# NthPortal/reservoir

Measured on AMD Instinct MI355X. Metric: elements sampled/sec (Gelem/s) + % HBM roofline, 1B Long keys k=1024, 1/2/4/8 GPU, higher is better.
Workload: dtype int64

## Files before the change

reservoir_amd/csrc/rsv_elements.hip:

```cpp
#include <algorithm>

#include "rsv_device.h"
#include "rsv_internal.h"
#include "rsv_scan.h"

namespace rsv {

namespace {

constexpr int kBlock = 256;

constexpr int kK1Unroll = 2;

constexpr unsigned kK1Grid = 256 * 20;

constexpr int kK1Win = 12;
struct K1Lds {
    uint64_t q[kBlock / 64][k1q_cap<kK1Win>()];
    uint64_t cq[kBlock / 64][kQueue];
};

__device__ __forceinline__ bool k1_fast(uint64_t lo, uint64_t hi) {
    return (lo >> 33) == ((hi - 1) >> 33) && hi <= (1ull << 40);
}

struct K1Sched {
    uint32_t W1, A, B;
};

__global__ __launch_bounds__(kBlock) void k1_last_writer(DrawKey dk, uint32_t k, uint64_t lo,
                                                         uint64_t hi, uint64_t g_begin,
                                                         uint64_t n_groups,
                                                         unsigned long long* __restrict__ win, K1Sched sch) {
    __shared__ K1Lds L;
    const int w = threadIdx.x >> 6;
    if (k1_fast(lo, hi))
        k1_body_q<kK1Win, true>(dk, k, lo, hi, g_begin, n_groups, win, L.q[w], L.cq[w], sch.W1, sch.A, sch.B);
    else
        k1_body_q<kK1Win, false>(dk, k, lo, hi, g_begin, n_groups, win, L.q[w], L.cq[w], sch.W1, sch.A, sch.B);
}

template <typename Take, typename Empty, typename Keep>
__device__ __forceinline__ void slot_rule(int64_t j, unsigned long long wi, int64_t base, int64_t n, int fresh,
                                          Take&& take, Empty&& empty, Keep&& keep) {
    if (wi) take((int64_t)wi - base, (int64_t)wi, true);
    else if (j >= base && j < base + n) take(j - base, j, false);
    else if (fresh) empty((int64_t)-1);
    else keep();
}

template <typename KeyT, int R, bool kAgentWin>
__device__ __forceinline__ void resolve_registers_first(const KeyT* __restrict__ keys, int64_t base, int64_t n,
                                                        uint32_t k, unsigned long long* __restrict__ win,
                                                        KeyT* __restrict__ slot_key, int64_t* __restrict__ slot_idx,
                                                        int fresh, int64_t m, KeyT* dst, uint32_t* flag, uint32_t gen) {
    unsigned long long wi[R];
    KeyT v[R];
#pragma unroll
    for (int r = 0; r < R; ++r) {
        const uint32_t j = threadIdx.x + r * kBlock;
        if (j >= k) wi[r] = 0ull;
        else if (kAgentWin) wi[r] = __hip_atomic_load(&win[j], __ATOMIC_RELAXED, __HIP_MEMORY_SCOPE_AGENT);
        else wi[r] = win[j];
    }
#pragma unroll
    for (int r = 0; r < R; ++r) {
        const int64_t j = threadIdx.x + r * kBlock;
        if (j >= k) continue;
        KeyT x;
        slot_rule(
            j, wi[r], base, n, fresh, [&](int64_t off, int64_t, bool) { x = keys[off]; }, [&](int64_t) { x = 0; },
            [&] { x = slot_key[j]; });
        v[r] = x;
    }
#pragma unroll
    for (int r = 0; r < R; ++r) {
        const int64_t j = threadIdx.x + r * kBlock;
        if (j >= k) continue;
        const KeyT x = v[r];
        slot_rule(
            j, wi[r], base, n, fresh,
            [=](int64_t, int64_t idx, bool winner) {
                slot_key[j] = x;
                slot_idx[j] = idx;
                if (winner) win[j] = 0;
            },
            [=](int64_t idx) {
                slot_key[j] = 0;
                slot_idx[j] = idx;
            },
            [] {});
        if (j < m) dst[j] = x;
    }
    publish_flag(flag, gen);
}

constexpr uint32_t kK1FusedMaxK = 8 * kBlock;

template <typename KeyT>
__global__ __launch_bounds__(kBlock) void k1_resolve_publish(DrawKey dk, uint32_t k, uint64_t lo, uint64_t hi,
                                                             uint64_t g_begin, uint64_t n_groups,
                                                             unsigned long long* __restrict__ win,
                                                             uint32_t* ticket, const KeyT* __restrict__ keys,
                                                             int64_t base, int64_t n, KeyT* __restrict__ slot_key,
                                                             int64_t* __restrict__ slot_idx, int fresh, int64_t m,
                                                             KeyT* dst, uint32_t* flag, uint32_t gen, K1Sched sch) {
    __shared__ K1Lds L;
    __shared__ uint32_t last;
    const int w = threadIdx.x >> 6;
    if (k1_fast(lo, hi))
        k1_body_q<kK1Win, true>(dk, k, lo, hi, g_begin, n_groups, win, L.q[w], L.cq[w], sch.W1, sch.A, sch.B);
    else
        k1_body_q<kK1Win, false>(dk, k, lo, hi, g_begin, n_groups, win, L.q[w], L.cq[w], sch.W1, sch.A, sch.B);
    asm volatile("s_waitcnt vmcnt(0)" ::: "memory");
    __syncthreads();
    if (threadIdx.x == 0) {
        const uint32_t prev = __hip_atomic_fetch_add(ticket, 1u, __ATOMIC_RELAXED, __HIP_MEMORY_SCOPE_AGENT);
        last = prev == gridDim.x - 1;
        if (last) __hip_atomic_store(ticket, 0u, __ATOMIC_RELAXED, __HIP_MEMORY_SCOPE_AGENT);
    }
    __syncthreads();
    if (!last) return;
    __builtin_amdgcn_fence(__ATOMIC_ACQUIRE, "agent");
    resolve_registers_first<KeyT, kK1FusedMaxK / kBlock, true>(keys, base, n, k, win, slot_key, slot_idx, fresh, m, dst,
                                                               flag, gen);
}

template <typename KeyT, bool kPublish>
__global__ __launch_bounds__(kPublish ? 1024 : kBlock) void resolve_kernel(const KeyT* __restrict__ keys, int64_t base,
                                                                         int64_t n, uint32_t k,
                                                                         unsigned long long* __restrict__ win,
                                                                         KeyT* __restrict__ slot_key,
                                                                         int64_t* __restrict__ slot_idx, int fresh,
                                                                         int64_t m, KeyT* dst, uint32_t* flag,
                                                                         uint32_t gen) {
    const uint32_t stride = gridDim.x * blockDim.x;
    for (uint32_t j = blockIdx.x * blockDim.x + threadIdx.x; j < k; j += stride) {
        KeyT v = 0;
        slot_rule(
            j, win[j], base, n, fresh,
            [&](int64_t off, int64_t idx, bool winner) {
                slot_key[j] = v = keys[off];
                if (kPublish || slot_idx) slot_idx[j] = idx;
                if (winner) win[j] = 0;
            },
            [=](int64_t idx) {
                slot_key[j] = 0;
                if (kPublish || slot_idx) slot_idx[j] = idx;
            },
            [&] {
                if (kPublish) v = slot_key[j];
            });
        if (kPublish && (int64_t)j < m) dst[j] = v;
    }
    if (kPublish) publish_flag(flag, gen);
}

template <typename KeyT, int R>
__global__ __launch_bounds__(kBlock) void resolve_publish_small_kernel(const KeyT* __restrict__ keys, int64_t base,
                                                                       int64_t n, uint32_t k,
                                                                       unsigned long long* __restrict__ win,
                                                                       KeyT* __restrict__ slot_key,
                                                                       int64_t* __restrict__ slot_idx, int fresh,
                                                                       int64_t m, KeyT* dst, uint32_t* flag, uint32_t gen) {
    resolve_registers_first<KeyT, R, false>(keys, base, n, k, win, slot_key, slot_idx, fresh, m, dst, flag, gen);
}

__global__ __launch_bounds__(kBlock) void replay_kernel(const int64_t* __restrict__ ev_pos,
                                                        const int32_t* __restrict__ ev_slot,
                                                        int64_t n_events, uint32_t k,
                                                        unsigned long long* __restrict__ win) {
    const int64_t e = (int64_t)blockIdx.x * blockDim.x + threadIdx.x;
    if (e >= n_events) return;
    const int32_t s = ev_slot[e];
    const int64_t p = ev_pos[e];
    if (s >= 0 && (uint32_t)s < k && p >= 2) atomicMax(&win[s], (unsigned long long)(p - 1));
}

__global__ __launch_bounds__(kBlock) void export_draws_kernel(DrawKey dk, uint64_t i0, int64_t n,
                                                              uint64_t* __restrict__ out) {
    const int64_t t = (int64_t)blockIdx.x * blockDim.x + threadIdx.x;
    if (t >= n) return;
    const uint64_t i = i0 + (uint64_t)t;
    const u32x4 w = level0(dk, i >> 4);
    out[t] = exact_j(dk, i, level0_byte(w, (uint32_t)(i & 15)));
}

template <typename KeyT>
struct StridedParts {
    using Key = KeyT;
    const int64_t* idx;
    const KeyT* key;
    int64_t part_len;
    __device__ int64_t index(int32_t p, uint32_t j) const { return idx[(int64_t)p * part_len + j]; }
    __device__ void take(int32_t p, uint32_t j, KeyT* slot_key) const { slot_key[j] = key[(int64_t)p * part_len + j]; }
};

template <typename KeyT>
struct PackedRows {
    using Key = KeyT;
    const int64_t* rows;
    int64_t stride;
    uint32_t k;
    __device__ int64_t index(int32_t p, uint32_t j) const { return rows[(int64_t)p * stride + j]; }
    __device__ void take(int32_t p, uint32_t j, KeyT* slot_key) const {
        slot_key[j] = (KeyT)rows[(int64_t)p * stride + k + j];
    }
};

struct StridedWideParts {
    using Key = uint32_t;
    const int64_t* idx;
    const uint32_t* key;
    int64_t part_len;
    uint32_t words;
    __device__ int64_t index(int32_t p, uint32_t j) const { return idx[(int64_t)p * part_len + j]; }
    __device__ void take(int32_t p, uint32_t j, uint32_t* slot_key) const {
        const uint32_t* src = key + ((size_t)p * part_len + j) * words;
        for (uint32_t q = 0; q < words; ++q) slot_key[(size_t)j * words + q] = src[q];
    }
};

struct PackedWideRows {
    using Key = uint32_t;
    const int64_t* rows;
    int64_t stride;
    uint32_t k, words;
    __device__ int64_t index(int32_t p, uint32_t j) const { return rows[(int64_t)p * stride + j]; }
    __device__ void take(int32_t p, uint32_t j, uint32_t* slot_key) const {
        const uint32_t* src = (const uint32_t*)(rows + (int64_t)p * stride + k) + (size_t)j * words;
        for (uint32_t q = 0; q < words; ++q) slot_key[(size_t)j * words + q] = src[q];
    }
};

template <typename Src>
__device__ __forceinline__ int32_t merge_winner(const Src& src, int32_t parts, uint32_t j, int64_t& best) {
    int32_t from = -1;
    for (int32_t p = 0; p < parts; ++p) {
        const int64_t idx = src.index(p, j);
        if (idx > best) {
            best = idx;
            from = p;
        }
    }
    return from;
}

template <typename Src, bool kPublish>
__global__ __launch_bounds__(kPublish ? 1024 : kBlock) void merge_kernel(Src src, int32_t parts, uint32_t k,
                                                                       int64_t* __restrict__ slot_idx,
                                                                       typename Src::Key* __restrict__ slot_key,
                                                                       int64_t m, typename Src::Key* dst,
                                                                       uint32_t* flag, uint32_t gen) {
    const uint32_t stride = gridDim.x * blockDim.x;
    for (uint32_t j = blockIdx.x * blockDim.x + threadIdx.x; j < k; j += stride) {
        int64_t best = slot_idx[j];
        const int32_t from = merge_winner(src, parts, j, best);
        if (from >= 0) {
            slot_idx[j] = best;
            src.take(from, j, slot_key);
        }
        if (kPublish && (int64_t)j < m) dst[j] = slot_key[j];
    }
    if (kPublish) publish_flag(flag, gen);
}

template <typename KeyT>
__global__ __launch_bounds__(kBlock) void export_packed_kernel(const int64_t* __restrict__ slot_idx,
                                                               const KeyT* __restrict__ slot_key, uint32_t k,
                                                               int64_t* __restrict__ row) {
    const uint32_t j = blockIdx.x * blockDim.x + threadIdx.x;
    if (j >= k) return;
    row[j] = slot_idx[j];
    row[k + j] = (int64_t)slot_key[j];
}

__global__ __launch_bounds__(1024) void resolve_wide_kernel(const uint32_t* __restrict__ keys, int64_t base,
                                                            int64_t n, uint32_t k, uint32_t words,
                                                            unsigned long long* __restrict__ win,
                                                            uint32_t* __restrict__ slot_key,
                                                            int64_t* __restrict__ slot_idx, int fresh, int64_t m,
                                                            uint32_t* dst, uint32_t* flag, uint32_t gen) {
    const uint32_t stride = gridDim.x * blockDim.x;
    for (uint32_t j = blockIdx.x * blockDim.x + threadIdx.x; j < k; j += stride) {
        const uint32_t* src = nullptr;
        bool write = true;
        slot_rule(
            j, win[j], base, n, fresh,
            [&](int64_t off, int64_t idx, bool winner) {
                src = keys + (size_t)off * words;
                slot_idx[j] = idx;
                if (winner) win[j] = 0;
            },
            [=](int64_t idx) { slot_idx[j] = idx; }, [&] { write = false; });
        uint32_t* o = slot_key + (size_t)j * words;
        const bool out = dst && (int64_t)j < m;
        for (uint32_t q = 0; q < words; ++q) {
            const uint32_t v = src ? src[q] : (write ? 0u : o[q]);
            if (write) o[q] = v;
            if (out) dst[(size_t)j * words + q] = v;
        }
    }
    if (dst) publish_flag(flag, gen);
}

__global__ __launch_bounds__(kBlock) void export_packed_wide_kernel(const int64_t* __restrict__ slot_idx,
                                                                    const uint32_t* __restrict__ slot_key, uint32_t k,
                                                                    uint32_t words, int64_t* __restrict__ row) {
    const uint32_t j = blockIdx.x * blockDim.x + threadIdx.x;
    if (j >= k) return;
    row[j] = slot_idx[j];
    uint32_t* o = (uint32_t*)(row + k) + (size_t)j * words;
    for (uint32_t q = 0; q < words; ++q) o[q] = slot_key[(size_t)j * words + q];
}

inline DrawKey make_key(const DrawParams& dp) {
    return DrawKey{(uint32_t)dp.seed, (uint32_t)(dp.seed >> 32), (uint32_t)dp.stream,
                   (uint32_t)(dp.stream >> 32)};
}

inline unsigned grid_for(uint64_t items, unsigned cap = ~0u) {
    uint64_t b = (items + kBlock - 1) / kBlock;
    if (b < 1) b = 1;
    return (unsigned)(b < cap ? b : cap);
}

inline unsigned k1_grid(uint64_t n_groups) {
    constexpr uint64_t per_window = (uint64_t)kK1Unroll * kBlock * kK1Win;
    if (n_groups < per_window * 768) return grid_for((n_groups + kK1Unroll - 1) / kK1Unroll, kK1Grid);
    const uint64_t m = std::max<uint64_t>(1, (n_groups + per_window * kK1Grid / 2) / (per_window * kK1Grid));
    return (unsigned)std::max<uint64_t>(1, n_groups / (per_window * m));
}

constexpr uint32_t kK1W1 = 256 * 6 * (kBlock / 64);
inline unsigned k1_plan(uint64_t n_groups, K1Sched& sch) {
    sch = K1Sched{0, 0, 0};
    constexpr uint64_t UB = (uint64_t)kK1Unroll * 64 * (kK1Win / 2);
    const uint64_t units = (n_groups + UB - 1) / UB;
    const uint64_t A = (units * 755 / 1000 + kK1W1 / 2) / kK1W1;
    if (n_groups < (uint64_t)kK1Unroll * kBlock * kK1Win * 768 || A < 10) return k1_grid(n_groups);
    sch.W1 = kK1W1;
    sch.A = (uint32_t)A;
    sch.B = 2;
    const uint64_t rest = units - (uint64_t)kK1W1 * A;
    const uint64_t waves = kK1W1 + (rest + sch.B - 1) / sch.B;
    return (unsigned)((waves + kBlock / 64 - 1) / (kBlock / 64));
}

template <typename F>
hipError_t with_key_type(int key_width, F&& f) {
    if (key_width == 8) f(int64_t{});
    else f(int32_t{});
    return hipGetLastError();
}

inline unsigned one_group_threads(uint32_t k) {
    return std::min<unsigned>(1024, std::max<unsigned>(64, (k + 63) / 64 * 64));
}

}

hipError_t launch_k1_last_writer(const DrawParams& dp, uint32_t k, uint64_t lo, uint64_t hi,
                                 unsigned long long* batch_win, hipStream_t st) {
    if (hi <= lo) return hipSuccess;
    const uint64_t g_end = (hi + 15) >> 4;
    constexpr uint64_t kMaxGroups = 1ull << 31;
    uint64_t n_groups = 0;
    for (uint64_t g_begin = lo >> 4; g_begin < g_end; g_begin += n_groups) {
        const uint64_t g_wrap = ((g_begin >> 32) + 1) << 32;
        n_groups = std::min<uint64_t>(std::min<uint64_t>(g_end, g_wrap) - g_begin, kMaxGroups);
        K1Sched sch;
        const unsigned grid = k1_plan(n_groups, sch);
        hipLaunchKernelGGL(k1_last_writer, dim3(grid), dim3(kBlock), 0, st, make_key(dp), k, lo, hi,
                           g_begin, n_groups, batch_win, sch);
        hipError_t e = hipGetLastError();
        if (e != hipSuccess) return e;
    }
    return hipSuccess;
}

bool k1_fused_ok(uint64_t lo, uint64_t hi, uint32_t k, int key_width) {
    if (hi <= lo || k > kK1FusedMaxK || (key_width != 8 && key_width != 4)) return false;
    const uint64_t g_begin = lo >> 4, g_end = (hi + 15) >> 4;
    return g_end - g_begin <= (1ull << 31) && g_end <= ((g_begin >> 32) + 1) << 32;
}

hipError_t launch_k1_resolve_publish(const DrawParams& dp, uint64_t lo, uint64_t hi, const SlotBlock& sb,
                                     uint32_t* ticket, const Batch& b, const Publication& pub, hipStream_t st) {
    if (!k1_fused_ok(lo, hi, sb.k, sb.key_width)) return hipErrorInvalidValue;
    const uint64_t g_begin = lo >> 4, n_groups = ((hi + 15) >> 4) - g_begin;
    K1Sched sch;
    const unsigned grid = k1_plan(n_groups, sch);
    return with_key_type(sb.key_width, [&](auto t) {
        using T = decltype(t);
        hipLaunchKernelGGL(k1_resolve_publish<T>, dim3(grid), dim3(kBlock), 0, st, make_key(dp), sb.k, lo, hi, g_begin,
                           n_groups, sb.win, ticket, (const T*)b.keys, b.base, b.n, (T*)sb.slot_key, sb.slot_idx,
                           (int)b.fresh, pub.m, (T*)pub.dst, pub.flag, pub.gen, sch);
    });
}

hipError_t launch_resolve(const SlotBlock& sb, const Batch& b, const Publication& pub, hipStream_t st, bool small) {
    const uint32_t k = sb.k;
    if (sb.key_width > 8) {
        const unsigned grid = pub.dst ? 1 : grid_for(k, 256 * 64);
        hipLaunchKernelGGL(resolve_wide_kernel, dim3(grid), dim3(pub.dst ? one_group_threads(k) : kBlock), 0, st,
                           (const uint32_t*)b.keys, b.base, b.n, k, (uint32_t)sb.key_width / 4, sb.win,
                           (uint32_t*)sb.slot_key, sb.slot_idx, (int)b.fresh, pub.m, (uint32_t*)pub.dst, pub.flag,
                           pub.gen);
        return hipGetLastError();
    }
    return with_key_type(sb.key_width, [&](auto t) {
        using T = decltype(t);
        auto go = [&](auto kernel, unsigned grid, unsigned threads) {
            hipLaunchKernelGGL(kernel, dim3(grid), dim3(threads), 0, st, (const T*)b.keys, b.base, b.n, k, sb.win,
                               (T*)sb.slot_key, sb.slot_idx, (int)b.fresh, pub.m, (T*)pub.dst, pub.flag, pub.gen);
        };
        if (!pub.dst) go(resolve_kernel<T, false>, grid_for(k), kBlock);
        else if (!(small && k <= 8 * kBlock)) go(resolve_kernel<T, true>, 1, one_group_threads(k));
        else if (k <= 2 * kBlock) go(resolve_publish_small_kernel<T, 2>, 1, kBlock);
        else if (k <= 4 * kBlock) go(resolve_publish_small_kernel<T, 4>, 1, kBlock);
        else go(resolve_publish_small_kernel<T, 8>, 1, kBlock);
    });
}

__global__ __launch_bounds__(kBlock) void init_slots_kernel(uint8_t* slot_key, int key_width, int64_t* slot_idx,
                                                            unsigned long long* win, uint32_t k, uint32_t* ticket) {
    const uint64_t stride = (uint64_t)gridDim.x * blockDim.x;
    if (ticket && blockIdx.x == 0 && threadIdx.x == 0) *ticket = 0;
    for (uint64_t j = (uint64_t)blockIdx.x * blockDim.x + threadIdx.x; j < k; j += stride) {
        win[j] = 0;
        slot_idx[j] = -1;
        if (key_width == 8)
            ((int64_t*)slot_key)[j] = 0;
        else if (key_width == 4)
            ((int32_t*)slot_key)[j] = 0;
        else
            for (int q = 0; q < key_width / 4; ++q) ((uint32_t*)slot_key)[(size_t)j * (key_width / 4) + q] = 0;
    }
}

hipError_t launch_init_slots(const SlotBlock& sb, hipStream_t st, uint32_t* ticket) {
    hipLaunchKernelGGL(init_slots_kernel, dim3(grid_for(sb.k, 256 * 64)), dim3(kBlock), 0, st, (uint8_t*)sb.slot_key,
                       sb.key_width, sb.slot_idx, sb.win, sb.k, ticket);
    return hipGetLastError();
}

__global__ __launch_bounds__(1024) void publish_kernel(const uint32_t* __restrict__ src, uint32_t* dst,
                                                      int64_t words, uint32_t* flag, uint32_t gen) {
    const int64_t vecs = words >> 2;
    for (int64_t i = threadIdx.x; i < vecs; i += blockDim.x)
        ((uint4*)dst)[i] = ((const uint4*)src)[i];
    for (int64_t i = (vecs << 2) + threadIdx.x; i < words; i += blockDim.x) dst[i] = src[i];
    publish_flag(flag, gen);
}

__global__ __launch_bounds__(1024) void publish_multi_kernel(const uint32_t* __restrict__ src, uint32_t* dst,
                                                            int64_t words, uint32_t* flag, uint32_t gen,
                                                            uint32_t* ticket) {
    const int64_t vecs = words >> 2;
    const int64_t stride = (int64_t)gridDim.x * blockDim.x;
    const int64_t t0 = (int64_t)blockIdx.x * blockDim.x + threadIdx.x;
    for (int64_t i = t0; i < vecs; i += stride) ((uint4*)dst)[i] = ((const uint4*)src)[i];
    for (int64_t i = (vecs << 2) + t0; i < words; i += stride) dst[i] = src[i];
    asm volatile("s_waitcnt vmcnt(0)" ::: "memory");
    __syncthreads();
    if (threadIdx.x == 0) {
        __threadfence_system();
        const uint32_t prev = __hip_atomic_fetch_add(ticket, 1u, __ATOMIC_ACQ_REL, __HIP_MEMORY_SCOPE_AGENT);
        if (prev == gridDim.x - 1) {
            __hip_atomic_store(ticket, 0u, __ATOMIC_RELAXED, __HIP_MEMORY_SCOPE_AGENT);
            __threadfence_system();
            __hip_atomic_store(flag, gen, __ATOMIC_RELEASE, __HIP_MEMORY_SCOPE_SYSTEM);
        }
    }
}

hipError_t launch_publish_multi(const void* src, int64_t bytes, void* dst_host_dev, uint32_t* flag_dev, uint32_t gen,
                                uint32_t* ticket_dev, hipStream_t st) {
    const int64_t per = 32 * 1024;
    const unsigned grid = (unsigned)std::min<int64_t>(32, std::max<int64_t>(1, (bytes + per - 1) / per));
    hipLaunchKernelGGL(publish_multi_kernel, dim3(grid), dim3(1024), 0, st, (const uint32_t*)src,
                       (uint32_t*)dst_host_dev, bytes / 4, flag_dev, gen, ticket_dev);
    return hipGetLastError();
}

hipError_t launch_publish(const void* src, int64_t bytes, void* dst_host_dev, uint32_t* flag_dev, uint32_t gen,
                          hipStream_t st) {
    hipLaunchKernelGGL(publish_kernel, dim3(1), dim3(1024), 0, st, (const uint32_t*)src, (uint32_t*)dst_host_dev,
                       bytes / 4, flag_dev, gen);
    return hipGetLastError();
}

__device__ __forceinline__ int64_t resolve_index_slot(uint64_t j, int64_t base, int64_t n, unsigned long long* win,
                                                      int64_t* slot_idx, int fresh, uint8_t* slot_key, int key_width) {
    int64_t off = -1;
    slot_rule(
        (int64_t)j, win[j], base, n, fresh,
        [&](int64_t o, int64_t idx, bool winner) {
            slot_idx[j] = idx;
            if (winner) win[j] = 0;
            off = o;
        },
        [=](int64_t idx) {
            slot_idx[j] = idx;
            for (int q = 0; q < key_width; ++q) slot_key[j * key_width + q] = 0;
        },
        [] {});
    return off;
}

__global__ __launch_bounds__(kBlock) void resolve_indices_kernel(int64_t base, int64_t n, uint32_t k,
                                                                 unsigned long long* __restrict__ win,
                                                                 int64_t* __restrict__ slot_idx, int fresh,
                                                                 uint8_t* __restrict__ slot_key, int key_width,
                                                                 int64_t* __restrict__ offs) {
    const uint64_t stride = (uint64_t)gridDim.x * blockDim.x;
    for (uint64_t j = (uint64_t)blockIdx.x * blockDim.x + threadIdx.x; j < k; j += stride)
        offs[j] = resolve_index_slot(j, base, n, win, slot_idx, fresh, slot_key, key_width);
}

__global__ __launch_bounds__(kBlock) void fill_slots_kernel(const int64_t* __restrict__ offs, const uint8_t* __restrict__ keys,
                                                            uint32_t k, int key_width, uint8_t* __restrict__ slot_key) {
    const uint64_t stride = (uint64_t)gridDim.x * blockDim.x;
    for (uint64_t j = (uint64_t)blockIdx.x * blockDim.x + threadIdx.x; j < k; j += stride) {
        if (offs[j] < 0) continue;
        if (key_width == 8) ((int64_t*)slot_key)[j] = ((const int64_t*)keys)[j];
        else if (key_width == 4) ((int32_t*)slot_key)[j] = ((const int32_t*)keys)[j];
        else
            for (int q = 0; q < key_width; ++q) slot_key[j * key_width + q] = keys[j * key_width + q];
    }
}


constexpr uint32_t kIdxPublishMaxK = 8192;

__global__ __launch_bounds__(1024) void resolve_indices_publish_kernel(int64_t base, int64_t n, uint32_t k,
                                                                       unsigned long long* __restrict__ win,
                                                                       int64_t* __restrict__ slot_idx, int fresh,
                                                                       uint8_t* __restrict__ slot_key, int key_width,
                                                                       int64_t* __restrict__ offs, int64_t* offs_host,
                                                                       uint32_t* flag, uint32_t gen) {
    for (uint32_t j = threadIdx.x; j < k; j += blockDim.x) {
        const int64_t off = resolve_index_slot(j, base, n, win, slot_idx, fresh, slot_key, key_width);
        offs[j] = off;
        offs_host[j] = off;
    }
    publish_flag(flag, gen);
}

template <typename KeyT>
__global__ __launch_bounds__(1024) void fill_slots_publish_kernel(const int64_t* __restrict__ offs,
                                                                  const KeyT* __restrict__ keys, uint32_t k,
                                                                  KeyT* __restrict__ slot_key, int64_t m, KeyT* dst,
                                                                  uint32_t* flag, uint32_t gen) {
    for (uint32_t j = threadIdx.x; j < k; j += blockDim.x) {
        KeyT v;
        if (offs[j] >= 0) {
            v = keys[j];
            slot_key[j] = v;
        } else {
            v = slot_key[j];
        }
        if ((int64_t)j < m) dst[j] = v;
    }
    publish_flag(flag, gen);
}

bool resolve_indices_publish_ok(uint32_t k) { return k <= kIdxPublishMaxK; }

hipError_t launch_resolve_indices(const SlotBlock& sb, const Batch& b, int64_t* offs, const Publication& pub,
                                  hipStream_t st) {
    if (!pub.dst)
        hipLaunchKernelGGL(resolve_indices_kernel, dim3(grid_for(sb.k, 256 * 64)), dim3(kBlock), 0, st, b.base, b.n, sb.k,
                           sb.win, sb.slot_idx, (int)b.fresh, (uint8_t*)sb.slot_key, sb.key_width, offs);
    else if (!resolve_indices_publish_ok(sb.k))
        return hipErrorInvalidValue;
    else
        hipLaunchKernelGGL(resolve_indices_publish_kernel, dim3(1), dim3(one_group_threads(sb.k)), 0, st, b.base, b.n,
                           sb.k, sb.win, sb.slot_idx, (int)b.fresh, (uint8_t*)sb.slot_key, sb.key_width, offs,
                           (int64_t*)pub.dst, pub.flag, pub.gen);
    return hipGetLastError();
}

bool fill_slots_publish_ok(uint32_t k, int key_width) {
    return k <= kIdxPublishMaxK && (key_width == 4 || key_width == 8);
}

hipError_t launch_fill_slots(const int64_t* offs, const void* keys, const SlotBlock& sb, const Publication& pub,
                             hipStream_t st) {
    if (!pub.dst) {
        hipLaunchKernelGGL(fill_slots_kernel, dim3(grid_for(sb.k, 256 * 64)), dim3(kBlock), 0, st, offs,
                           (const uint8_t*)keys, sb.k, sb.key_width, (uint8_t*)sb.slot_key);
        return hipGetLastError();
    }
    if (!fill_slots_publish_ok(sb.k, sb.key_width)) return hipErrorInvalidValue;
    return with_key_type(sb.key_width, [&](auto t) {
        using T = decltype(t);
        hipLaunchKernelGGL(fill_slots_publish_kernel<T>, dim3(1), dim3(one_group_threads(sb.k)), 0, st, offs,
                           (const T*)keys, sb.k, (T*)sb.slot_key, pub.m, (T*)pub.dst, pub.flag, pub.gen);
    });
}

hipError_t launch_replay_events(const int64_t* ev_pos, const int32_t* ev_slot, int64_t n_events,
                                uint32_t k, unsigned long long* batch_win, hipStream_t st) {
    if (n_events <= 0) return hipSuccess;
    const unsigned grid = (unsigned)((n_events + kBlock - 1) / kBlock);
    hipLaunchKernelGGL(replay_kernel, dim3(grid), dim3(kBlock), 0, st, ev_pos, ev_slot, n_events, k,
                       batch_win);
    return hipGetLastError();
}

hipError_t launch_export_draws(const DrawParams& dp, uint64_t i0, int64_t n, uint64_t* j,
                               hipStream_t st) {
    if (n <= 0) return hipSuccess;
    const unsigned grid = (unsigned)((n + kBlock - 1) / kBlock);
    hipLaunchKernelGGL(export_draws_kernel, dim3(grid), dim3(kBlock), 0, st, make_key(dp), i0, n, j);
    return hipGetLastError();
}

namespace {

template <bool kPublish, typename Src>
void launch_merge(const Src& src, int32_t parts, const SlotBlock& sb, const Publication& pub, hipStream_t st) {
    using Key = typename Src::Key;
    hipLaunchKernelGGL((merge_kernel<Src, kPublish>), dim3(kPublish ? 1 : grid_for(sb.k)),
                       dim3(kPublish ? one_group_threads(sb.k) : kBlock), 0, st, src, parts, sb.k, sb.slot_idx,
                       (Key*)sb.slot_key, pub.m, (Key*)pub.dst, pub.flag, pub.gen);
}

}

hipError_t launch_merge_slots(const int64_t* idx_parts, const void* key_parts, int32_t parts, int64_t part_len,
                              const SlotBlock& sb, hipStream_t st) {
    if (sb.key_width > 8) {
        const StridedWideParts src{idx_parts, (const uint32_t*)key_parts, part_len, (uint32_t)sb.key_width / 4};
        launch_merge<false>(src, parts, sb, Publication{}, st);
        return hipGetLastError();
    }
    return with_key_type(sb.key_width, [&](auto t) {
        using T = decltype(t);
        launch_merge<false>(StridedParts<T>{idx_parts, (const T*)key_parts, part_len}, parts, sb, Publication{}, st);
    });
}

hipError_t launch_export_packed(const SlotBlock& sb, int64_t* row, hipStream_t st) {
    if (sb.key_width > 8) {
        hipLaunchKernelGGL(export_packed_wide_kernel, dim3(grid_for(sb.k)), dim3(kBlock), 0, st, sb.slot_idx,
                           (const uint32_t*)sb.slot_key, sb.k, (uint32_t)sb.key_width / 4, row);
        return hipGetLastError();
    }
    return with_key_type(sb.key_width, [&](auto t) {
        using T = decltype(t);
        hipLaunchKernelGGL(export_packed_kernel<T>, dim3(grid_for(sb.k)), dim3(kBlock), 0, st, sb.slot_idx,
                           (const T*)sb.slot_key, sb.k, row);
    });
}

hipError_t launch_merge_packed(const int64_t* rows, int32_t parts, int64_t stride, const SlotBlock& sb,
                               const Publication& pub, hipStream_t st) {
    if (sb.key_width > 8) {
        if (pub.dst) return hipErrorInvalidValue;
        launch_merge<false>(PackedWideRows{rows, stride, sb.k, (uint32_t)sb.key_width / 4}, parts, sb, pub, st);
        return hipGetLastError();
    }
    return with_key_type(sb.key_width, [&](auto t) {
        using T = decltype(t);
        const PackedRows<T> src{rows, stride, sb.k};
        if (pub.dst) launch_merge<true>(src, parts, sb, pub, st);
        else launch_merge<false>(src, parts, sb, pub, st);
    });
}

}
```

reservoir_amd/csrc/rsv_scan.h:

```cpp
#pragma once
#include <algorithm>

#include "rsv_device.h"

namespace rsv {

constexpr uint32_t kQueue = 128;
constexpr uint64_t kIndexMask = (1ull << 56) - 1;

__device__ __forceinline__ uint32_t clip_mask16(uint64_t i0, uint64_t lo, uint64_t hi) {
    uint32_t m = 0xFFFFu;
    if (i0 < lo) m = (lo - i0 >= 16) ? 0u : ((0xFFFFu << (uint32_t)(lo - i0)) & 0xFFFFu);
    if (i0 + 16 > hi) m &= (hi <= i0) ? 0u : (0xFFFFu >> (uint32_t)(16 - (hi - i0)));
    return m;
}

__device__ __forceinline__ uint32_t candidate_mask16(const u32x4& w, uint64_t i0, uint64_t dense_lim) {
    if (i0 + 1 >= dense_lim) return zero_byte_mask16(w);
    const float Tf = __fdividef((float)dense_lim, (float)(i0 + 1));
    if (Tf > 300.0f) return 0xFFFFu;
    uint32_t T = (uint32_t)Tf;
    if ((uint64_t)T * (i0 + 1) < dense_lim) ++T;
    if (T > 0 && (uint64_t)(T - 1) * (i0 + 1) >= dense_lim) --T;
    return lt_mask16(w, T > 256u ? 256u : T);
}

template <class Hit>
__device__ __forceinline__ void resolve_entry(const DrawKey& dk, uint64_t e, uint32_t k, Hit& hit) {
    const uint64_t i = e & kIndexMask;
    const uint64_t j = exact_j(dk, i, (uint32_t)(e >> 56));
    if (j < k) hit((uint32_t)j, i);
}

template <class Hit>
__device__ __forceinline__ void enqueue_block(const DrawKey& dk, const u32x4& w, uint64_t i0,
                                              uint32_t mask, uint64_t* q, uint32_t& qn,
                                              uint32_t lane, uint32_t k, Hit& hit) {
    while (__any(mask != 0)) {
        const bool has = mask != 0;
        const unsigned long long bal = __ballot(has);
        if (has) {
            const uint32_t e = __builtin_ctz(mask);
            mask &= mask - 1;
            q[qn + __popcll(bal & lanemask_lt64())] = ((uint64_t)level0_byte(w, e) << 56) | (i0 + e);
        }
        qn += (uint32_t)__popcll(bal);
        if (qn >= 64) {
            qn -= 64;
            __builtin_amdgcn_wave_barrier();
            resolve_entry(dk, q[qn + lane], k, hit);
            __builtin_amdgcn_wave_barrier();
        }
    }
}

template <class Hit>
__device__ __forceinline__ void drain_queue(const DrawKey& dk, const uint64_t* q, uint32_t& qn,
                                            uint32_t lane, uint32_t k, Hit& hit) {
    __builtin_amdgcn_wave_barrier();
    if (lane < qn) resolve_entry(dk, q[lane], k, hit);
    qn = 0;
    __builtin_amdgcn_wave_barrier();
}


template <class Hit>
__device__ __forceinline__ void resolve_block(const DrawKey& dk, bool valid, uint64_t g, uint64_t lo,
                                              uint64_t hi, uint64_t dense_lim, uint32_t k, uint64_t* cq,
                                              uint32_t& cqn, uint32_t lane, Hit& hit) {
    const u32x4 w = level0(dk, g);
    const uint64_t i0 = g << 4;
    uint32_t mask = valid ? candidate_mask16(w, i0, dense_lim) : 0u;
    if (i0 < lo || i0 + 16 > hi) mask &= clip_mask16(i0, lo, hi);
    if (mask) {
        const uint32_t e = __builtin_ctz(mask);
        mask &= mask - 1;
        const uint64_t j = exact_j(dk, i0 + e, level0_byte(w, e));
        if (j < k) hit((uint32_t)j, i0 + e);
    }
    enqueue_block(dk, w, i0, mask, cq, cqn, lane, k, hit);
}

__device__ __forceinline__ uint32_t fold16(const u32x4& w) {
    const uint32_t x = w.x | w.y | w.z | w.w;
    uint32_t y;
    asm("v_or_b32_sdwa %0, %1, %1 dst_sel:WORD_0 dst_unused:UNUSED_PAD src0_sel:WORD_0 src1_sel:WORD_1\n\t"
        "s_nop 0"
        : "=v"(y)
        : "v"(x));
    return y;
}

__device__ __forceinline__ u32x4 level1_b0_words(const DrawKey& dk, uint64_t i, bool hi_uniform, uint32_t c1u) {
    const uint64_t g1 = i >> 1;
    if (hi_uniform) return philox4x32_10_uniform_hi((uint32_t)g1, c1u, dk.s0, dk.s1, dk.k0, dk.k1);
    return philox4x32_10((uint32_t)g1, (uint32_t)(g1 >> 32) | kDomainLevel1, dk.s0, dk.s1, dk.k0, dk.k1);
}

__device__ __forceinline__ uint32_t fold_pair(const u32x4& a, const u32x4& b) {
    const uint32_t xa = a.x | a.y | a.z | a.w, xb = b.x | b.y | b.z | b.w;
    uint32_t z;
    asm("v_or_b32_sdwa %0, %1, %1 dst_sel:WORD_0 dst_unused:UNUSED_PAD src0_sel:WORD_0 src1_sel:WORD_1\n\t"
        "s_nop 0\n\t"
        "v_or_b32_sdwa %0, %2, %2 dst_sel:WORD_1 dst_unused:UNUSED_PRESERVE src0_sel:WORD_0 src1_sel:WORD_1\n\t"
        "s_nop 0"
        : "=&v"(z)
        : "v"(xa), "v"(xb));
    return z;
}

template <int W>
constexpr uint32_t k1q_cap() { return 64u * (1u + W / 2); }
constexpr uint32_t kQueueWaves = 4;

template <int W = 12, bool FAST = false>
__device__ __forceinline__ void k1_body_q(const DrawKey& dk, uint32_t k, uint64_t lo, uint64_t hi, uint64_t g_begin,
                                          uint64_t n_groups, unsigned long long* __restrict__ win, uint64_t* q,
                                          uint64_t* cq, uint32_t W1 = 0, uint32_t A = 0, uint32_t B = 0,
                                          uint32_t* pool = nullptr) {
    static_assert(W % 2 == 0, "half windows");
    constexpr int U = 2;
    const uint32_t lane = threadIdx.x & 63;
    uint32_t qn = 0, cqn = 0;
    auto hit = [&](uint32_t j, uint64_t i) { atomicMax(&win[j], (unsigned long long)i); };
    const uint64_t dense_lim = 256ull * k;
    const uint32_t ng = (uint32_t)n_groups;
    const uint64_t g_sparse = (dense_lim + 14) >> 4;
    const uint32_t off_sparse = g_sparse <= g_begin ? 0u : (uint32_t)std::min<uint64_t>(g_sparse - g_begin, ng);
    const uint32_t stride = gridDim.x * blockDim.x * U;
    const uint32_t c1u = (uint32_t)__builtin_amdgcn_readfirstlane((int)((uint32_t)(lo >> 33) | kDomainLevel1));
    const bool hi_uniform = (lo >> 33) == ((hi - 1) >> 33);
    const bool pre_ok = hi <= (1ull << 40);
    const uint64_t k_hi = (uint64_t)k << 32, k_24 = (uint64_t)k << 24;
    int32_t dpend = 0;
    const uint32_t g0 = (uint32_t)g_begin;
    uint32_t base = __builtin_amdgcn_readfirstlane((blockIdx.x * blockDim.x + (threadIdx.x & ~63u)) * U);
    const uint32_t ghi = (uint32_t)__builtin_amdgcn_readfirstlane((int)(uint32_t)(g_begin >> 32));
    uint32_t gl = g0 + base + lane;
    const uint32_t off_steady =
        __builtin_amdgcn_readfirstlane((int)std::max<uint32_t>(off_sparse, (lo & 15) ? 1u : 0u));
    const uint32_t ng_steady = __builtin_amdgcn_readfirstlane((int)(ng - ((hi & 15) ? 1u : 0u)));

    auto resolve = [&](bool valid, uint64_t ent) {
        const uint32_t gt = (uint32_t)ent * kPhiloxM0Inv, off = gt - g0, z = (uint32_t)(ent >> 32);
        __builtin_assume(!valid || z != 0xFFFFFFFFu);
        bool dense = false;
        if (dpend > 0) {
            dense = valid && ((z & 0xFFFFu) == 0 || (z >> 16) == 0);
            const unsigned long long db = __builtin_amdgcn_ballot_w64(dense);
            if (db) {
                resolve_block(dk, dense, g_begin + off, lo, hi, dense_lim, k, cq, cqn, lane, hit);
                resolve_block(dk, dense && off + 64 < ng, g_begin + off + 64, lo, hi, dense_lim, k, cq, cqn, lane, hit);
                dpend -= std::min<int32_t>(dpend, (int32_t)__popcll(db));
            }
        }
        const uint32_t zm = (valid && !dense) ? ~z : 0u;
        uint32_t rest = 0;
        if (zm) {
            const uint32_t e = __builtin_ctz(zm);
            rest = zm & (zm - 1);
            if constexpr (FAST) {
                const uint32_t bl = gt + ((e & 16u) << 2);
                const uint32_t g1lo = (bl << 3) | ((e & 15u) >> 1);
                const u32x4 w = philox4x32_10_uniform_hi(g1lo, c1u, dk.s0, dk.s1, dk.k0, dk.k1);
                const bool odd = e & 1u;
                const uint32_t Lh = odd ? w.z : w.x;
                const uint32_t i8 = (ghi << 28) | (bl >> 4);
                if ((uint64_t)(Lh >> 8) * i8 < k_24) {
                    const uint64_t i = ((((uint64_t)ghi << 32) | bl) << 4) | (e & 15u);
                    const uint64_t L = ((uint64_t)Lh << 32) | (odd ? w.w : w.y);
                    const uint64_t j = __umul64hi(L >> 8, i + 1);
                    if (j < k) hit((uint32_t)j, i);
                }
            } else {
                const uint64_t i = ((g_begin + off + ((e >> 4) << 6)) << 4) + (e & 15u);
                const u32x4 w = level1_b0_words(dk, i, hi_uniform, c1u);
                const uint32_t Lh = (i & 1) ? w.z : w.x;
                const bool maybe = !pre_ok || (uint64_t)(Lh >> 8) * (i + 1) < k_hi;
                if (maybe) {
                    const uint64_t L = ((uint64_t)Lh << 32) | ((i & 1) ? w.w : w.y);
                    const uint64_t j = __umul64hi(L >> 8, i + 1);
                    if (j < k) hit((uint32_t)j, i);
                }
            }
        }
        const unsigned long long bal = __builtin_amdgcn_ballot_w64(rest != 0);
        if (bal) {
            if (rest) {
                const uint32_t pos = __builtin_amdgcn_mbcnt_hi((uint32_t)(bal >> 32), __builtin_amdgcn_mbcnt_lo((uint32_t)bal, 0u));
                q[qn + pos] = (uint64_t)(uint32_t)ent | ((uint64_t)~rest << 32);
            }
            qn += (uint32_t)__popcll(bal);
        }
    };
    auto rounds = [&]() {
        while (qn >= 64) {
            qn -= 64;
            __builtin_amdgcn_wave_barrier();
            const uint64_t ent = q[qn + lane];
            __builtin_amdgcn_wave_barrier();
            resolve(true, ent);
            __builtin_amdgcn_wave_barrier();
        }
    };
    auto append = [&](bool has, uint32_t gt, uint32_t z) {
        const unsigned long long bal = __builtin_amdgcn_ballot_w64(has);
        if (has) {
            const uint32_t pos = __builtin_amdgcn_mbcnt_hi((uint32_t)(bal >> 32), __builtin_amdgcn_mbcnt_lo((uint32_t)bal, 0u));
            q[qn + pos] = (uint64_t)gt | ((uint64_t)z << 32);
        }
        qn += (uint32_t)__popcll(bal);
    };

    const uint32_t q_s = (uint32_t)__builtin_amdgcn_readfirstlane((int)(uint32_t)(uintptr_t)q);
    uint32_t m0v;
    asm volatile("v_mov_b32 %0, %1" : "=v"(m0v) : "s"(kPhiloxM0));
    auto steady = [&](uint32_t d) {
        u32x4 w0, w1;
        uint32_t glo;
        philox4x32_10_uniform_hi_x2_at(gl, m0v, (uint64_t)kPhiloxM0 * d, ghi, dk.s0, dk.s1, dk.k0, dk.k1, w0, w1, glo);
        const uint32_t xa = w0.x | w0.y | w0.z | w0.w, xb = w1.x | w1.y | w1.z | w1.w;
        uint32_t z;
        unsigned long long m;
        asm("v_or_b32_sdwa %0, %2, %2 dst_sel:WORD_0 dst_unused:UNUSED_PAD src0_sel:WORD_0 src1_sel:WORD_1\n\t"
            "s_nop 0\n\t"
            "v_or_b32_sdwa %0, %3, %3 dst_sel:WORD_1 dst_unused:UNUSED_PRESERVE src0_sel:WORD_0 src1_sel:WORD_1\n\t"
            "s_nop 0\n\t"
            "v_cmp_ne_u32_e64 %1, -1, %0"
            : "=&v"(z), "=s"(m)
            : "v"(xa), "v"(xb));
        const uint32_t pos = __builtin_amdgcn_mbcnt_hi((uint32_t)(m >> 32), __builtin_amdgcn_mbcnt_lo((uint32_t)m, 0u));
        const uint32_t sb = q_s + 8u * qn;
        const uint64_t ent = (uint64_t)glo | ((uint64_t)z << 32);
        unsigned long long sv;
        uint32_t addr;
        asm volatile("v_lshl_add_u32 %1, %2, 3, %3\n\t"
                     "s_mov_b64 %0, exec\n\t"
                     "s_mov_b64 exec, %4\n\t"
                     "ds_write_b64 %1, %5\n\t"
                     "s_mov_b64 exec, %0"
                     : "=&s"(sv), "=&v"(addr)
                     : "v"(pos), "s"(sb), "s"(m), "v"(ent)
                     : "memory");
        qn += (uint32_t)__popcll(m);
    };
    auto partial = [&](uint32_t b) {
        u32x4 w[U];
#pragma unroll
        for (int u = 0; u < U; ++u)
            w[u] = philox4x32_10_uniform_hi(gl, ghi, dk.s0, dk.s1, dk.k0, dk.k1, (uint64_t)kPhiloxM0 * (64u * u));
        uint32_t z;
        bool has;
        if (b >= off_steady && b + U * 64 <= ng_steady) {
            z = fold_pair(w[0], w[1]);
            has = z != 0xFFFFFFFFu;
        } else {
            uint32_t y[U];
            bool hb[U];
#pragma unroll
            for (int u = 0; u < U; ++u) {
                const uint32_t off = b + u * 64 + lane;
                const uint64_t i0 = (g_begin + off) << 4;
                const bool dense = i0 + 1 < dense_lim;
                y[u] = off >= ng ? 0xFFFFu
                                 : dense ? 0u : (fold16(w[u]) | (~clip_mask16(i0, lo, hi) & 0xFFFFu));
                hb[u] = (off < ng) & (dense | ((uint16_t)y[u] != 0xFFFFu));
            }
            z = (y[0] & 0xFFFFu) | (y[1] << 16);
            has = hb[0] | hb[1];
        }
        dpend += (int32_t)__popcll(__builtin_amdgcn_ballot_w64(has && ((z & 0xFFFFu) == 0 || (z >> 16) == 0)));
        append(has, gl * kPhiloxM0, z);
        __builtin_amdgcn_wave_barrier();
        rounds();
    };
    if (A > 0) {
        constexpr uint32_t UB = (W / 2) * U * 64;
        const uint32_t units = (ng + UB - 1) / UB;
        const uint32_t wg = __builtin_amdgcn_readfirstlane((blockIdx.x * blockDim.x + threadIdx.x) >> 6);
        const uint32_t nB = gridDim.x * (blockDim.x >> 6) - W1;
        const bool ga = wg < W1;
        const uint32_t cnt = ga ? A : B, u_step = ga ? W1 : nB, u_first = ga ? wg : W1 * A + (wg - W1);
        for (uint32_t j = 0; j < cnt; ++j) {
            const uint32_t u = u_first + j * u_step;
            if (u >= units) break;
            uint32_t ub = u * UB;
            gl = g0 + ub + lane;
            if (ub >= off_steady && ub + UB <= ng_steady) {
#pragma unroll
                for (int t = 0; t < W / 2; ++t) steady(t * (U * 64));
                __builtin_amdgcn_wave_barrier();
                rounds();
            } else {
                for (int t = 0; t < W / 2 && ub < ng; ++t, ub += U * 64, gl += U * 64) partial(ub);
            }
        }
        base = ng;
    }
    while (base < ng) {
        if (base >= off_steady && (uint64_t)base + (uint64_t)(W - 1) * stride + U * 64 <= ng_steady) {
#pragma unroll
            for (int h = 0; h < 2; ++h) {
#pragma unroll
                for (int t = 0; t < W / 2; ++t) steady(t * stride);
                gl += (W / 2) * stride;
                __builtin_amdgcn_wave_barrier();
                rounds();
            }
            base += W * stride;
        } else {
            for (int t = 0; t < W && base < ng; ++t, base += stride, gl += stride) {
                partial(base);
            }
        }
    }
    if (pool) {
        constexpr uint32_t cap = k1q_cap<W>(), NW = kQueueWaves;
        const uint32_t wv = threadIdx.x >> 6;
        const uint64_t* q0 = q - (size_t)wv * cap;
        for (;;) {
            if (lane == 0) pool[wv] = qn | (dpend > 0 ? 0x80000000u : 0u);
            __syncthreads();
            uint32_t c[NW], T = 0, anyd = 0;
#pragma unroll
            for (uint32_t v = 0; v < NW; ++v) {
                const uint32_t pv = (uint32_t)__builtin_amdgcn_readfirstlane((int)pool[v]);
                c[v] = pv & 0x7FFFFFFFu;
                anyd |= pv >> 31;
                T += c[v];
            }
            if (T == 0) break;
            uint32_t o = 64u * wv + lane, src = 0;
            const bool valid = o < T;
#pragma unroll
            for (uint32_t v = 0; v + 1 < NW; ++v)
                if (src == v && o >= c[v]) {
                    o -= c[v];
                    src = v + 1;
                }
            const uint64_t ent = valid ? q0[(size_t)src * cap + o] : 0ull;
            __syncthreads();
            qn = 0;
            dpend = anyd ? (1 << 30) : 0;
            if (64u * wv < T) resolve(valid, ent);
        }
    } else {
        while (qn > 0) {
            __builtin_amdgcn_wave_barrier();
            const uint32_t nv = std::min<uint32_t>(qn, 64u);
            qn -= nv;
            const bool valid = lane < nv;
            const uint64_t ent = valid ? q[qn + lane] : 0ull;
            __builtin_amdgcn_wave_barrier();
            resolve(valid, ent);
        }
    }
    __builtin_amdgcn_wave_barrier();
    drain_queue(dk, cq, cqn, lane, k, hit);
}

}
```

Before: 11490.

## Precompute k1 launch parameters on host and split head/tail from steady units

Moves per-kernel scalar setup (sparse offsets, steady bounds, stride, flags, k shifts) into a host-computed K1Launch struct passed as a kernel argument. The scheduled path now aligns steady units after the head, so the unit loop always runs the unrolled steady body with no boundary branch. Head and tail partial iterations are handed to the first W1 waves. The A/rest split is also retuned to a fixed remainder, and queue positions now come from the mbcnt intrinsic instead of a popcount of a lane mask. The cost is a larger kernel argument block and more load on the first-wave group, which could unbalance the schedule.

```diff
diff --git a/reservoir_amd/csrc/rsv_elements.hip b/reservoir_amd/csrc/rsv_elements.hip
--- a/reservoir_amd/csrc/rsv_elements.hip
+++ b/reservoir_amd/csrc/rsv_elements.hip
@@ -20,24 +20,14 @@
     uint64_t cq[kBlock / 64][kQueue];
 };
 
-__device__ __forceinline__ bool k1_fast(uint64_t lo, uint64_t hi) {
-    return (lo >> 33) == ((hi - 1) >> 33) && hi <= (1ull << 40);
-}
-
-struct K1Sched {
-    uint32_t W1, A, B;
-};
-
 __global__ __launch_bounds__(kBlock) void k1_last_writer(DrawKey dk, uint32_t k, uint64_t lo,
                                                          uint64_t hi, uint64_t g_begin,
                                                          uint64_t n_groups,
-                                                         unsigned long long* __restrict__ win, K1Sched sch) {
+                                                         unsigned long long* __restrict__ win, K1Launch P) {
     __shared__ K1Lds L;
     const int w = threadIdx.x >> 6;
-    if (k1_fast(lo, hi))
-        k1_body_q<kK1Win, true>(dk, k, lo, hi, g_begin, n_groups, win, L.q[w], L.cq[w], sch.W1, sch.A, sch.B);
-    else
-        k1_body_q<kK1Win, false>(dk, k, lo, hi, g_begin, n_groups, win, L.q[w], L.cq[w], sch.W1, sch.A, sch.B);
+    if (P.flags & kK1Fast) k1_body_q<kK1Win, true, kBlock>(dk, k, lo, hi, g_begin, n_groups, win, L.q[w], L.cq[w], P);
+    else k1_body_q<kK1Win, false, kBlock>(dk, k, lo, hi, g_begin, n_groups, win, L.q[w], L.cq[w], P);
 }
 
 template <typename Take, typename Empty, typename Keep>
@@ -104,14 +94,12 @@
                                                              uint32_t* ticket, const KeyT* __restrict__ keys,
                                                              int64_t base, int64_t n, KeyT* __restrict__ slot_key,
                                                              int64_t* __restrict__ slot_idx, int fresh, int64_t m,
-                                                             KeyT* dst, uint32_t* flag, uint32_t gen, K1Sched sch) {
+                                                             KeyT* dst, uint32_t* flag, uint32_t gen, K1Launch P) {
     __shared__ K1Lds L;
     __shared__ uint32_t last;
     const int w = threadIdx.x >> 6;
-    if (k1_fast(lo, hi))
-        k1_body_q<kK1Win, true>(dk, k, lo, hi, g_begin, n_groups, win, L.q[w], L.cq[w], sch.W1, sch.A, sch.B);
-    else
-        k1_body_q<kK1Win, false>(dk, k, lo, hi, g_begin, n_groups, win, L.q[w], L.cq[w], sch.W1, sch.A, sch.B);
+    if (P.flags & kK1Fast) k1_body_q<kK1Win, true, kBlock>(dk, k, lo, hi, g_begin, n_groups, win, L.q[w], L.cq[w], P);
+    else k1_body_q<kK1Win, false, kBlock>(dk, k, lo, hi, g_begin, n_groups, win, L.q[w], L.cq[w], P);
     asm volatile("s_waitcnt vmcnt(0)" ::: "memory");
     __syncthreads();
     if (threadIdx.x == 0) {
@@ -333,18 +321,13 @@
 }
 
 constexpr uint32_t kK1W1 = 256 * 6 * (kBlock / 64);
-inline unsigned k1_plan(uint64_t n_groups, K1Sched& sch) {
-    sch = K1Sched{0, 0, 0};
-    constexpr uint64_t UB = (uint64_t)kK1Unroll * 64 * (kK1Win / 2);
-    const uint64_t units = (n_groups + UB - 1) / UB;
-    const uint64_t A = (units * 755 / 1000 + kK1W1 / 2) / kK1W1;
-    if (n_groups < (uint64_t)kK1Unroll * kBlock * kK1Win * 768 || A < 10) return k1_grid(n_groups);
-    sch.W1 = kK1W1;
-    sch.A = (uint32_t)A;
-    sch.B = 2;
-    const uint64_t rest = units - (uint64_t)kK1W1 * A;
-    const uint64_t waves = kK1W1 + (rest + sch.B - 1) / sch.B;
-    return (unsigned)((waves + kBlock / 64 - 1) / (kBlock / 64));
+constexpr uint32_t kK1Rest = 5400, kK1MinA = 5;
+inline unsigned k1_plan(uint32_t k, uint64_t lo, uint64_t hi, uint64_t g_begin, uint64_t n_groups, K1Launch& P) {
+    const unsigned stride_grid = k1_grid(n_groups);
+    P = k1_launch<kK1Win>(k, lo, hi, g_begin, n_groups, stride_grid, kBlock);
+    if (P.units < kK1MinA * kK1W1 + kK1Rest) return stride_grid;
+    const unsigned grid = k1_schedule(P, kK1W1, (P.units - kK1Rest) / kK1W1, 2, kBlock);
+    return grid ? grid : stride_grid;
 }
 
 template <typename F>
@@ -369,10 +352,10 @@
     for (uint64_t g_begin = lo >> 4; g_begin < g_end; g_begin += n_groups) {
         const uint64_t g_wrap = ((g_begin >> 32) + 1) << 32;
         n_groups = std::min<uint64_t>(std::min<uint64_t>(g_end, g_wrap) - g_begin, kMaxGroups);
-        K1Sched sch;
-        const unsigned grid = k1_plan(n_groups, sch);
+        K1Launch P;
+        const unsigned grid = k1_plan(k, lo, hi, g_begin, n_groups, P);
         hipLaunchKernelGGL(k1_last_writer, dim3(grid), dim3(kBlock), 0, st, make_key(dp), k, lo, hi,
-                           g_begin, n_groups, batch_win, sch);
+                           g_begin, n_groups, batch_win, P);
         hipError_t e = hipGetLastError();
         if (e != hipSuccess) return e;
     }
@@ -389,13 +372,13 @@
                                      uint32_t* ticket, const Batch& b, const Publication& pub, hipStream_t st) {
     if (!k1_fused_ok(lo, hi, sb.k, sb.key_width)) return hipErrorInvalidValue;
     const uint64_t g_begin = lo >> 4, n_groups = ((hi + 15) >> 4) - g_begin;
-    K1Sched sch;
-    const unsigned grid = k1_plan(n_groups, sch);
+    K1Launch P;
+    const unsigned grid = k1_plan(sb.k, lo, hi, g_begin, n_groups, P);
     return with_key_type(sb.key_width, [&](auto t) {
         using T = decltype(t);
         hipLaunchKernelGGL(k1_resolve_publish<T>, dim3(grid), dim3(kBlock), 0, st, make_key(dp), sb.k, lo, hi, g_begin,
                            n_groups, sb.win, ticket, (const T*)b.keys, b.base, b.n, (T*)sb.slot_key, sb.slot_idx,
-                           (int)b.fresh, pub.m, (T*)pub.dst, pub.flag, pub.gen, sch);
+                           (int)b.fresh, pub.m, (T*)pub.dst, pub.flag, pub.gen, P);
     });
 }
 
diff --git a/reservoir_amd/csrc/rsv_scan.h b/reservoir_amd/csrc/rsv_scan.h
--- a/reservoir_amd/csrc/rsv_scan.h
+++ b/reservoir_amd/csrc/rsv_scan.h
@@ -42,7 +42,8 @@
         if (has) {
             const uint32_t e = __builtin_ctz(mask);
             mask &= mask - 1;
-            q[qn + __popcll(bal & lanemask_lt64())] = ((uint64_t)level0_byte(w, e) << 56) | (i0 + e);
+            const uint32_t pos = __builtin_amdgcn_mbcnt_hi((uint32_t)(bal >> 32), __builtin_amdgcn_mbcnt_lo((uint32_t)bal, 0u));
+            q[qn + pos] = ((uint64_t)level0_byte(w, e) << 56) | (i0 + e);
         }
         qn += (uint32_t)__popcll(bal);
         if (qn >= 64) {
@@ -113,11 +114,66 @@
 constexpr uint32_t k1q_cap() { return 64u * (1u + W / 2); }
 constexpr uint32_t kQueueWaves = 4;
 
-template <int W = 12, bool FAST = false>
+
+constexpr uint32_t kK1Fast = 1u, kK1HiUniform = 2u, kK1Below2p40 = 4u;
+struct K1Launch {
+    uint32_t W1, A, B;
+    uint32_t nB;
+    uint32_t units;
+    uint32_t unit_off;
+    uint32_t head_iters;
+    uint32_t slow_iters;
+    uint32_t tail_off;
+    uint32_t stride;
+    uint32_t off_steady, ng_steady;
+    uint32_t c1u, ghi;
+    uint32_t flags;
+    uint64_t k24, khi;
+};
+
+template <int W = 12>
+inline K1Launch k1_launch(uint32_t k, uint64_t lo, uint64_t hi, uint64_t g_begin, uint64_t n_groups, unsigned grid,
+                          unsigned block = 256) {
+    constexpr uint32_t UB = (W / 2) * 2 * 64, IB = 2 * 64;
+    K1Launch P{};
+    const uint32_t ng = (uint32_t)n_groups;
+    const uint64_t g_sparse = (256ull * k + 14) >> 4;
+    const uint32_t off_sparse = g_sparse <= g_begin ? 0u : (uint32_t)std::min<uint64_t>(g_sparse - g_begin, ng);
+    P.off_steady = std::max<uint32_t>(off_sparse, (lo & 15) ? 1u : 0u);
+    P.ng_steady = ng - ((hi & 15) ? 1u : 0u);
+    P.stride = grid * block * 2;
+    P.c1u = (uint32_t)(lo >> 33) | kDomainLevel1;
+    P.ghi = (uint32_t)(g_begin >> 32);
+    const bool hi_uniform = (lo >> 33) == ((hi - 1) >> 33), below = hi <= (1ull << 40);
+    P.flags = (hi_uniform && below ? kK1Fast : 0u) | (hi_uniform ? kK1HiUniform : 0u) | (below ? kK1Below2p40 : 0u);
+    P.k24 = (uint64_t)k << 24;
+    P.khi = (uint64_t)k << 32;
+    const uint32_t head = (uint32_t)std::min<uint64_t>(((uint64_t)P.off_steady + IB - 1) / IB * IB, ng);
+    P.unit_off = head;
+    P.units = P.ng_steady > head ? (P.ng_steady - head) / UB : 0u;
+    P.tail_off = head + P.units * UB;
+    P.head_iters = (head + IB - 1) / IB;
+    P.slow_iters = P.head_iters + (ng - P.tail_off + IB - 1) / IB;
+    return P;
+}
+
+inline unsigned k1_schedule(K1Launch& P, uint32_t W1, uint32_t A, uint32_t B, unsigned block = 256) {
+    if (W1 == 0 || A == 0 || B == 0 || (uint64_t)W1 * A >= P.units) return 0;
+    const uint64_t rest = P.units - (uint64_t)W1 * A;
+    const uint64_t wpg = block / 64, waves = W1 + (rest + B - 1) / B;
+    const unsigned grid = (unsigned)((waves + wpg - 1) / wpg);
+    P.W1 = W1;
+    P.A = A;
+    P.B = B;
+    P.nB = (uint32_t)(grid * wpg - W1);
+    P.stride = grid * block * 2;
+    return grid;
+}
+
+template <int W = 12, bool FAST = false, int BS = 256>
 __device__ __forceinline__ void k1_body_q(const DrawKey& dk, uint32_t k, uint64_t lo, uint64_t hi, uint64_t g_begin,
                                           uint64_t n_groups, unsigned long long* __restrict__ win, uint64_t* q,
-                                          uint64_t* cq, uint32_t W1 = 0, uint32_t A = 0, uint32_t B = 0,
-                                          uint32_t* pool = nullptr) {
+                                          uint64_t* cq, const K1Launch& P, uint32_t* pool = nullptr) {
     static_assert(W % 2 == 0, "half windows");
     constexpr int U = 2;
     const uint32_t lane = threadIdx.x & 63;
@@ -125,21 +181,17 @@
     auto hit = [&](uint32_t j, uint64_t i) { atomicMax(&win[j], (unsigned long long)i); };
     const uint64_t dense_lim = 256ull * k;
     const uint32_t ng = (uint32_t)n_groups;
-    const uint64_t g_sparse = (dense_lim + 14) >> 4;
-    const uint32_t off_sparse = g_sparse <= g_begin ? 0u : (uint32_t)std::min<uint64_t>(g_sparse - g_begin, ng);
-    const uint32_t stride = gridDim.x * blockDim.x * U;
-    const uint32_t c1u = (uint32_t)__builtin_amdgcn_readfirstlane((int)((uint32_t)(lo >> 33) | kDomainLevel1));
-    const bool hi_uniform = (lo >> 33) == ((hi - 1) >> 33);
-    const bool pre_ok = hi <= (1ull << 40);
-    const uint64_t k_hi = (uint64_t)k << 32, k_24 = (uint64_t)k << 24;
+    const uint32_t stride = P.stride;
+    const uint32_t c1u = P.c1u;
+    const bool hi_uniform = P.flags & kK1HiUniform;
+    const bool pre_ok = P.flags & kK1Below2p40;
+    const uint64_t k_hi = P.khi, k_24 = P.k24;
     int32_t dpend = 0;
     const uint32_t g0 = (uint32_t)g_begin;
-    uint32_t base = __builtin_amdgcn_readfirstlane((blockIdx.x * blockDim.x + (threadIdx.x & ~63u)) * U);
-    const uint32_t ghi = (uint32_t)__builtin_amdgcn_readfirstlane((int)(uint32_t)(g_begin >> 32));
+    uint32_t base = __builtin_amdgcn_readfirstlane((blockIdx.x * BS + (threadIdx.x & ~63u)) * U);
+    const uint32_t ghi = P.ghi;
     uint32_t gl = g0 + base + lane;
-    const uint32_t off_steady =
-        __builtin_amdgcn_readfirstlane((int)std::max<uint32_t>(off_sparse, (lo & 15) ? 1u : 0u));
-    const uint32_t ng_steady = __builtin_amdgcn_readfirstlane((int)(ng - ((hi & 15) ? 1u : 0u)));
+    const uint32_t off_steady = P.off_steady, ng_steady = P.ng_steady;
 
     auto resolve = [&](bool valid, uint64_t ent) {
         const uint32_t gt = (uint32_t)ent * kPhiloxM0Inv, off = gt - g0, z = (uint32_t)(ent >> 32);
@@ -274,26 +326,27 @@
         __builtin_amdgcn_wave_barrier();
         rounds();
     };
-    if (A > 0) {
+    if (P.A > 0) {
         constexpr uint32_t UB = (W / 2) * U * 64;
-        const uint32_t units = (ng + UB - 1) / UB;
-        const uint32_t wg = __builtin_amdgcn_readfirstlane((blockIdx.x * blockDim.x + threadIdx.x) >> 6);
-        const uint32_t nB = gridDim.x * (blockDim.x >> 6) - W1;
+        const uint32_t W1 = P.W1;
+        const uint32_t wg = __builtin_amdgcn_readfirstlane((blockIdx.x * BS + threadIdx.x) >> 6);
         const bool ga = wg < W1;
-        const uint32_t cnt = ga ? A : B, u_step = ga ? W1 : nB, u_first = ga ? wg : W1 * A + (wg - W1);
+        if (ga) {
+            for (uint32_t d = wg; d < P.slow_iters; d += W1) {
+                const uint32_t b = d < P.head_iters ? d * (U * 64) : P.tail_off + (d - P.head_iters) * (U * 64);
+                gl = g0 + b + lane;
+                partial(b);
+            }
+        }
+        const uint32_t cnt = ga ? P.A : P.B, u_step = ga ? W1 : P.nB, u_first = ga ? wg : W1 * P.A + (wg - W1);
         for (uint32_t j = 0; j < cnt; ++j) {
             const uint32_t u = u_first + j * u_step;
-            if (u >= units) break;
-            uint32_t ub = u * UB;
-            gl = g0 + ub + lane;
-            if (ub >= off_steady && ub + UB <= ng_steady) {
-#pragma unroll
-                for (int t = 0; t < W / 2; ++t) steady(t * (U * 64));
-                __builtin_amdgcn_wave_barrier();
-                rounds();
-            } else {
-                for (int t = 0; t < W / 2 && ub < ng; ++t, ub += U * 64, gl += U * 64) partial(ub);
-            }
+            if (u >= P.units) break;
+            gl = g0 + P.unit_off + u * UB + lane;
+#pragma unroll
+            for (int t = 0; t < W / 2; ++t) steady(t * (U * 64));
+            __builtin_amdgcn_wave_barrier();
+            rounds();
         }
         base = ng;
     }
```

Result: faster. 11660, median of 6 (+1.5%).
